# AvilaAndre/simgrid-flow-updating-implementation

Hardware: AMD Instinct MI355X
Metric: directed-edge flow updates/sec + % HBM roofline; rounds to 1e-9 error (higher is better)
Workload: dtype f64

## Files before the change

### simgrid-flow-updating-implementation_amd/csrc/fu_engine.hip

```cpp
#include <hip/hip_runtime.h>
#include <hip/hip_ext.h>

#include <algorithm>
#include <cmath>
#include <cstring>
#include <string>
#include <vector>

#include "fu_common.h"
#include "fu_plan.h"

using namespace fu;
namespace FP = fu::plan;

#define HIP_TRY(expr)                                                                     \
  do {                                                                                    \
    hipError_t _e = (expr);                                                               \
    if (_e != hipSuccess)                                                                 \
      return fu::fail(FU_ERR_HIP, std::string(#expr) + ": " + hipGetErrorString(_e));     \
  } while (0)

namespace {

using FP::kGeoEdges;
// ... 876 lines not shown
  const int excl = base + x - (len[0] + len[1]);
  if (2 * t < P) {
    s_m[2 * t] = excl;
    s_o[2 * t] = o[0];
  }
  if (2 * t + 1 < P) {
    s_m[2 * t + 1] = excl + len[0];
    s_o[2 * t + 1] = o[1];
  }
  if (t == 0) {
    int tot = 0;
    for (int k = 0; k < kTrThreads / 64; ++k) tot += s_w[k];
    s_m[P] = tot;
  }
  __syncthreads();
  const int nst = s_m[P];
  if (t < kTrBE / 64) {
    const int m = t * 64;
    int lo = 1, hi = P;
    while (lo < hi) {
      const int mid = (lo + hi) >> 1;
      if (s_m[mid] > m) hi = mid; else lo = mid + 1;
    }
    s_c[t] = lo;
  }
  if (t == 0) s_c[kTrBE / 64] = P;
  __syncthreads();
  constexpr int kPerT = kTrBE / kTrThreads;
  int g[kPerT];
#pragma unroll
  for (int k = 0; k < kPerT; ++k) {
    const int m = t + k * kTrThreads;
    g[k] = -1;
    if (m < nst) {
      int lo = s_c[m >> 6], hi = s_c[(m >> 6) + 1];
      while (lo < hi) {
        const int mid = (lo + hi) >> 1;
        if (s_m[mid] > m) hi = mid; else lo = mid + 1;
      }
      const int run = lo - 1;
      g[k] = s_o[run] + (m - s_m[run]);
    }
  }
  double val[kPerT];
  unsigned short pos[kPerT];
#pragma unroll
  for (int k = 0; k < kPerT; ++k) {
    val[k] = g[k] >= 0 ? GA[g[k]] : 0.0;
    pos[k] = g[k] >= 0 ? pos16[g[k]] : (unsigned short)0;
  }
  const int next = bk + nj;
  if (next < bend) load_runs(next, o, len);
#pragma unroll
  for (int k = 0; k < kPerT; ++k)
    if (g[k] >= 0) s_v[pos[k]] = val[k];
  __syncthreads();
  for (int q = t; q < ne; q += kTrThreads) {
    if constexpr (NT) __builtin_nontemporal_store(s_v[q], GB + e0 + q);
    else GB[e0 + q] = s_v[q];
  }
  if (next >= bend) break;
  __syncthreads();
  bk = next;
  }
}

__global__ __launch_bounds__(kBlock) void k_isolated(int i0, int n, const double *__restrict__ v,
                                                     double *__restrict__ a_new, const double *__restrict__ target,
                                                     unsigned long long *__restrict__ err, void *__restrict__ code_new,
                                                     PackCtl *__restrict__ ctl, int rslot, int check) {
  const PackCtl pc = ctl[2];
  if (blockIdx.x == 0 && threadIdx.x == 0) ctl[rslot] = pc;
  const int i = i0 + blockIdx.x * kBlock + threadIdx.x;
  unsigned long long eb = 0;
  if (i < n) {
    const double a = ((v[i] - 0.0) + 0.0) / (double)1;
    *(a_new + i) = a;
    if (pc.width) put_code(pc, code_new, i, a);
    if (check) eb = err_bits(a, target[i]);
  }
  if (check) block_max_to(eb, err);
}

template <bool CHECK, int TE, int TN, bool RF = true, bool LO = true>
__global__ __launch_bounds__(kBlock) void k_round_staged(
    const int4 *__restrict__ tiles, int t0, int ntl,
    const int *__restrict__ rowptr, const int *__restrict__ col,
    const StageArgs sa, const void *__restrict__ G, const double *__restrict__ v,
    double *__restrict__ F, const double *__restrict__ a_prev, const double *__restrict__ a_prev2,
    double *__restrict__ a_new, const double *__restrict__ target,
    unsigned long long *__restrict__ err, void *__restrict__ code_new, PackCtl *__restrict__ ctl,
    int rslot, int fm) {
  static_assert(TE % kBlock == 0 && TN <= kBlock, "tile geometry");
  static_assert(TE <= 1024, "the u16 staged index holds a 10-bit tile position");
  const PackCtl pp = ctl[rslot ^ 1];
  const int lsel = sa.sel[width_index(pp.width)];
  const PackCtl pc = ctl[2];
  if (blockIdx.x == 0 && threadIdx.x == 0) ctl[rslot] = pc;
  __shared__ double s_x[TE];
  __shared__ double s_er[TE];
  __shared__ unsigned char s_own[TE];
  __shared__ int s_rp[TN + 1];
  __shared__ double s_a[TN];
  const int t = threadIdx.x;
  unsigned long long eb = 0;
  const int xcd = blockIdx.x & 7, per = ntl >> 3, rem = ntl & 7;
  const int tile = t0 + xcd * per + min(xcd, rem) + (int)(blockIdx.x >> 3);
  const int4 tl = tiles[tile];
  const int nb = tl.x, nn = tl.y - tl.x;
  const int e0 = tl.z, ne = tl.w - tl.z;
  constexpr int kPer = TE / kBlock;
  const unsigned short *__restrict__ s16 = sa.sidx16[lsel];
  unsigned si[kPer];
  double x[kPer], g[kPer];
  int gi[kPer];
  int rp;
  double vv, own2;
  if constexpr (LO) {
  {
    const int dl = sa.dtab[lsel][(size_t)tile * kStageRuns + (t & 63)];
    unsigned short c16[kPer];
#pragma unroll
    for (int k = 0; k < kPer; ++k) {
      const int q = t + k * kBlock;
      const unsigned short c = s16[q < ne ? e0 + q : 0];
      c16[k] = q < ne ? c : (unsigned short)0;
    }
    if constexpr (RF) {
#pragma unroll
      for (int k = 0; k < kPer; ++k) {
        const int q = t + k * kBlock;
        const double f = ld_f(F, q < ne ? e0 + q : 0);
        x[k] = q < ne ? f : 0.0;
      }
    } else {
#pragma unroll
      for (int k = 0; k < kPer; ++k) x[k] = 0.0;
    }
    const int tn = min(t, nn - 1);
    const int rp0 = rowptr[nb + min(t, nn)];
    const double v0 = v[nb + tn], o0 = a_prev2[nb + tn];
    asm volatile("" ::: "memory");
    rp = t <= nn ? rp0 : 0;
    vv = t < nn ? v0 : 0.0;
    own2 = t < nn ? o0 : 0.0;
#pragma unroll
    for (int k = 0; k < kPer; ++k) {
      const int q = t + k * kBlock;
      const int dd = __shfl(dl, (int)(c16[k] >> 10));
      si[k] = c16[k] & 1023u;
      gi[k] = q < ne ? q + dd : -1;
    }
  }
  } else {
  {
    const int dl = sa.dtab[lsel][(size_t)tile * kStageRuns + (t & 63)];
    unsigned short c16[kPer];
#pragma unroll
    for (int k = 0; k < kPer; ++k) {
      const int q = t + k * kBlock;
      c16[k] = q < ne ? s16[e0 + q] : (unsigned short)0;
      x[k] = q < ne && RF ? ld_f(F, e0 + q) : 0.0;
    }
#pragma unroll
    for (int k = 0; k < kPer; ++k) {
      const int q = t + k * kBlock;
      const int dd = __shfl(dl, (int)(c16[k] >> 10));
      si[k] = c16[k] & 1023u;
      gi[k] = q < ne ? q + dd : -1;
    }
  }
  rp = t <= nn ? rowptr[nb + t] : 0;
  vv = t < nn ? v[nb + t] : 0.0;
  own2 = t < nn ? a_prev2[nb + t] : 0.0;
  }
  if (pp.width == 0) {
#pragma unroll
    for (int k = 0; k < kPer; ++k)
      g[k] = gi[k] >= 0 ? reinterpret_cast<const double *>(G)[gi[k]] : 0.0;
  } else {
    unsigned cd[kPer];
    unsigned esc;
    if (pp.width == 8) {
      esc = 0xFFu;
#pragma unroll
      for (int k = 0; k < kPer; ++k) cd[k] = gi[k] >= 0 ? reinterpret_cast<const unsigned char *>(G)[gi[k]] : 0u;
    } else if (pp.width == 16) {
      esc = 0xFFFFu;
#pragma unroll
      for (int k = 0; k < kPer; ++k) cd[k] = gi[k] >= 0 ? reinterpret_cast<const unsigned short *>(G)[gi[k]] : 0u;
    } else {
      esc = 0xFFFFFFFFu;
#pragma unroll
      for (int k = 0; k < kPer; ++k) cd[k] = gi[k] >= 0 ? reinterpret_cast<const unsigned *>(G)[gi[k]] : 0u;
    }
#pragma unroll
    for (int k = 0; k < kPer; ++k)
      g[k] = gi[k] < 0 ? 0.0 : cd[k] == esc ? a_prev[col[e0 + (int)(si[k] & 0xFFFFu)]] : dkey_inv(pp.base + cd[k]);
  }
#pragma unroll
  for (int k = 0; k < kPer; ++k) {
    const int q = t + k * kBlock;
    if (q < ne) {
      s_x[q] = x[k];
      s_er[si[k] & 0xFFFFu] = g[k];
    }
  }
  if (t <= nn) s_rp[t] = rp;
  __syncthreads();
  if (t < nn) {
    const int qb = s_rp[t] - e0, qe = s_rp[t + 1] - e0;
    double S = 0.0, T = 0.0;
    const double fo0 = fm ? old_flow(fm, own2) : 0.0;
    for (int q = qb; q < qe; ++q) {
      const double er = s_er[q];
      const double fr = recon_fr(fm ? fo0 : s_x[q], er, own2);
      s_x[q] = fr;
      s_own[q] = (unsigned char)t;
      S = S + fr;
      T = T + er;
    }
    const double a = ((vv - S) + T) / (double)(qe - qb + 1);
    s_a[t] = a;
    *(a_new + nb + t) = a;
    if (pc.width) put_code(pc, code_new, nb + t, a);
    if (CHECK) eb = err_bits(a, target[nb + t]);
  }
  __syncthreads();
#pragma unroll
  for (int k = 0; k < kPer; ++k) {
    const int q = t + k * kBlock;
    if (q < ne) {
      st_fo(F, e0 + q, (s_x[q] + s_a[s_own[q]]) - s_er[q], x[k], fm);
    }
  }
  if (CHECK) block_max_to(eb, err);
}


constexpr int kMCH = 64;
template <bool CHECK, int LAGM = 0>
__global__ __launch_bounds__(kBlock) void k_heavy_multi(
    const int *__restrict__ hrows, int nrows, const int *__restrict__ rowptr, const double *__restrict__ v,
    double *__restrict__ F, const double *__restrict__ a_prev2, double *__restrict__ a_new,
    const double *__restrict__ target, unsigned long long *__restrict__ err, void *__restrict__ code_new,
    PackCtl *__restrict__ ctl, const double *__restrict__ Gb, int fm,
    const double *__restrict__ Gb_old = nullptr, double *__restrict__ hist = nullptr) {
  constexpr bool LAG = LAGM > 0;
  constexpr bool mat = LAGM == 2;
  __shared__ double sh[2][2 * kMR][kMCH + 1];
  __shared__ int s_b[kMR], s_d[kMR];
  __shared__ double s_o2[kMR], s_a[kMR], s_o4[kMR];
  const PackCtl pc = ctl[2];
  const int t = threadIdx.x, w = t >> 6, lane = t & 63;
  const int r0 = blockIdx.x * kMR;
  if (t < kMR) {
    const bool ok = r0 + t < nrows;
    const int i = ok ? hrows[r0 + t] : 0;
    const int b = ok ? rowptr[i] : 0;
    s_b[t] = b;
    s_d[t] = ok ? rowptr[i + 1] - b : 0;
    const double o2 = ok ? a_prev2[i] : 0.0;
    s_o2[t] = o2;
    if (LAG) {
      s_o4[t] = ok && mat ? hist[r0 + t] : 0.0;
      if (ok) hist[r0 + t] = o2;
    }
  }
  __syncthreads();
  int rb[4], rd[4];
  double ro2[4], ro4[4];
#pragma unroll
  for (int j = 0; j < 4; ++j) {
    rb[j] = s_b[4 * w + j];
    rd[j] = s_d[4 * w + j];
    ro2[j] = s_o2[4 * w + j];
    ro4[j] = LAG ? s_o4[4 * w + j] : 0.0;
  }
  const int nch = (s_d[0] + kMCH - 1) / kMCH;
  double fo0[4], er0[4], fo1[4], er1[4];
  double eo0[4], eo1[4];
  auto load = [&](double (&fo)[4], double (&er)[4], double (&eo)[4], int c) {
#pragma unroll
    for (int j = 0; j < 4; ++j) {
      const int k = min(c * kMCH + lane, max(rd[j] - 1, 0));
      er[j] = Gb[rb[j] + k];
      if constexpr (mat) eo[j] = Gb_old[rb[j] + k];
      if constexpr (mat) fo[j] = ld_f(F, rb[j] + k);
      else fo[j] = ld_fo(F, rb[j] + k, fm, ro2[j]);
    }
  };
  auto put = [&](const double (&fo)[4], const double (&er)[4], const double (&eo)[4], int c, int buf) {
#pragma unroll
    for (int j = 0; j < 4; ++j) {
      const int r = 4 * w + j;
      const bool in = c * kMCH + lane < rd[j];
      double f2 = fo[j];
      if (LAG && in) {
        const int e = rb[j] + c * kMCH + lane;
        if constexpr (mat) {
          f2 = (recon_fr(fo[j], eo[j], ro4[j]) + ro2[j]) - eo[j];
          st_f(F, e, f2, fo[j]);
        } else if (fm) {
          st_f_full(F, e, f2);
        }
      }
      sh[buf][2 * r][lane] = in ? recon_fr(f2, er[j], ro2[j]) : 0.0;
      sh[buf][2 * r + 1][lane] = in ? er[j] : 0.0;
    }
  };
  const int cr = lane >> 1, ch = lane & 1;
  double acc = 0.0;
  auto chain = [&](int c, int buf) {
    if (w == 0 && lane < 2 * kMR) {
      const int len = min(kMCH, max(0, s_d[cr] - c * kMCH));
      const double *src = sh[buf][lane];
      int q = 0;
// ... 553 lines not shown
    if (++it > max_iters) {
      atomicExch(status, 1);
      break;
    }
  }
  if (done)
    while (sc < n_snap && snap_ticks[sc] < tick_end) snaps[(long long)sc++ * n + node] = lst;
#pragma unroll
  for (int j = 0; j < MAXD; ++j)
    if (j < deg) {
      flow[rb + j] = fl[j];
      est[rb + j] = es[j];
    }
  cursor[node] = p;
  scur[node] = sc;
  last[node] = lst;
}
#undef FU_RING_REFILL
#undef FU_RING_COMMIT
#undef FU_NEXT_RECVS


template <typename T>
int dmalloc(T **p, size_t count) {
  if (count == 0) count = 1;
  hipError_t e = hipMalloc((void **)p, sizeof(T) * count);
  if (e != hipSuccess) {
    *p = nullptr;
    return fail(FU_ERR_ALLOC, std::string("hipMalloc(") + std::to_string(sizeof(T) * count) + "): " + hipGetErrorString(e));
  }
  return FU_OK;
}

}

struct RoundCtx {
  int64_t r;
  int fm;
  double *F;
  const double *ap, *ap2;
  double *an;
  unsigned long long *err;
  bool plan;
};

constexpr int kPreMarks = 12;

struct fu_handle {
  int device = 0;
  std::vector<int32_t> h_new_of_old;
  std::vector<int64_t> h_orig_rowptr;
  hipStream_t stream = nullptr;
  hipStream_t stream2 = nullptr;
  hipEvent_t ev0 = nullptr, ev1 = nullptr;
  hipEvent_t ev2 = nullptr, ev3 = nullptr;
  hipEvent_t marks[64] = {};
  hipEvent_t r0_start = nullptr;
  hipEvent_t r0_stop = nullptr;
  hipEvent_t ev_pw = nullptr, ev_fork = nullptr, ev_join = nullptr;
  int32_t n = 0;
  int64_t E = 0;
  int32_t na = 0;
  int32_t max_deg = 0;
  int *rowptr = nullptr, *col = nullptr;
  int *blk_row = nullptr;
  unsigned short *col16 = nullptr;
  int *cbase = nullptr;
  std::vector<int32_t> h_cbase;
  double *v = nullptr;
  double *f[2] = {nullptr, nullptr};
  double *a[3] = {nullptr, nullptr, nullptr};
  double *target = nullptr;
  unsigned long long *err = nullptr;
  int errcap = 0;
  double *ftmp = nullptr;
  int64_t rounds = 0;
  int kernel = 4;
  int geo = 1;
  int hub_threshold = 128;
  int mega_hub = 8192;
  int wave_heavy = 1;
  int mid_heavy = 1;
  int tr_bpx = 32;
  int staged_lo = 1;
  int c16 = 1;
  int multi_mid = 1;
  int split_hubs = 1;
  int fork_heavy = 1;
  bool autotune = true;
  bool tuned = false;
  bool tune_for_width = false;
  bool tuning = false;
  float tune_ms[8] = {};
  int tune_out[8] = {};
  int n_tunes = 0;
  int tuned_width = 0;
  int tune_cache[4] = {-1, -1, -1, -1};
  int *h_pw = nullptr;
  void *h_xfer[2] = {nullptr, nullptr};
  hipEvent_t ev_xfer[2] = {nullptr, nullptr};
  bool pw_pending = false;
  int *pw_dev = nullptr;
  bool plan_pending = false;
  std::vector<int64_t> h_rowptr;
  std::vector<int32_t> h_col;
  int4 *tiles_geo[4] = {nullptr, nullptr, nullptr, nullptr};
  int *tnar_geo[4] = {nullptr, nullptr, nullptr, nullptr};
  int ntiles_geo[4] = {0, 0, 0, 0};
  int nheavy_geo[4] = {0, 0, 0, 0};
  int nbound_geo[4] = {0, 0, 0, 0};
  int niso_geo[4] = {0, 0, 0, 0};
  int iso0_geo[4] = {0, 0, 0, 0};
  FP::Tiles tiles1;
  int mid_geo[4][2] = {};
  int multi_geo[4][2] = {};
  int multi_heavy = 1;
  double *halo_a = nullptr;
  std::vector<int32_t> h_hrows;
  int *hrows = nullptr;
  int n_hub = 0;
  int64_t hub_total = 0;
  int4 *hub_rows = nullptr;
  int *hub_blk = nullptr;
  int iso_rows = 1;
  int multi_short = 1;
  int tr_nt = 1;
  int *hub_off = nullptr;
  double2 *hubxy = nullptr;
  unsigned char *code[2] = {nullptr, nullptr};
  PackCtl *pctl = nullptr;
  int *psample = nullptr;
  int n_psample = 0;
  int pack = 1;
  int pack_every = 16;
  int tile_edges = 1024;
  int tile_nodes = 0;
  bool has_target = false;
  struct StageLayout {
    int P = 0, Q = 0, SN = 0, NB = 0;
    int4 *brange = nullptr;
    unsigned short *colS = nullptr;
    unsigned short *sidx16 = nullptr;
    int *dtab = nullptr;
  };
  StageLayout st[4];
  bool st_ready = false;
  std::string st_why;
  int4 *st_tiles = nullptr;
  int st_ntiles = 0;
  int st_nbound = 0;
  int4 *st_heavy = nullptr;
  int st_nheavy = 0;
  void *stG = nullptr;
  int seen_width = 0;
  int st_force = -1;
  std::vector<FP::I4> h_light;
  struct TransLayout {
    int P = 0, Q = 0, NB = 0, B = 0;
    int Bh = 0;
    int Bm = 0;
    int4 *brange = nullptr;
    unsigned short *colS = nullptr;
    unsigned short *pos16 = nullptr;
    int *offT = nullptr;
    double *GA = nullptr;
    double *GBr[3] = {nullptr, nullptr, nullptr};
    double *hist[2] = {nullptr, nullptr};
// ... 218 lines not shown
  T.Bm = tp.Bm;
  h->tr_ready = true;
  return FU_OK;
}

inline unsigned grid_for(long long work) { return (unsigned)((work + kBlock - 1) / kBlock); }

int lag_finalize(fu_handle *h, int p) {
  if (!h->lagf[p]) return FU_OK;
  const int64_t rr = h->lag_round[p];
  if (h->rounds - rr < 1 || h->rounds - rr > 2)
    return fail(FU_ERR_STATE, "lag_finalize: lagged round " + std::to_string(rr) + " is not one of the last two (" +
                                  std::to_string(h->rounds) + " rounds done)");
  const double *Gb = h->tr.GBr[rr % 3];
  const double *a = h->a[rr % 3];
  if (h->lag_nmulti[p])
    hipLaunchKernelGGL(k_lag_final, dim3(h->lag_nmulti[p]), dim3(kBlock), 0, h->stream, h->hrows + h->multi_geo[1][0],
                       h->rowptr, h->f[p], Gb, h->tr.hist[p], a);
  HIP_TRY(hipGetLastError());
  h->lagf[p] = 0;
  return FU_OK;
}
int lag_finalize_all(fu_handle *h) {
  for (int p = 0; p < 2; ++p)
    if (int rc = lag_finalize(h, p)) return rc;
  return FU_OK;
}

inline unsigned tr_grid(fu_handle *h, int nbk) {
  const int per = (nbk + 7) / 8;
  return 8u * (unsigned)(h->tr_bpx > 0 ? std::min(per, h->tr_bpx) : per);
}


void plan_alone(fu_handle *h, RoundCtx &c) {
  if (!c.plan) return;
  hipLaunchKernelGGL(k_pack_plan, dim3(1), dim3(kBlock), 0, h->stream, c.ap, h->psample, h->pctl, h->pw_dev);
  c.plan = false;
}

int launch_round0(fu_handle *h, RoundCtx &c) {
  static_assert(sizeof(PackCtl) * 3 == 6 * sizeof(unsigned long long), "k_round0 clears 3 PackCtl");
  h->lagf[0] = h->lagf[1] = 0;
  if (h->r0_start) {
    hipExtLaunchKernelGGL(k_round0, dim3(grid_for(std::max(h->na, 6))), dim3(kBlock), 0, h->stream, h->r0_start,
                          h->r0_stop, 0, h->n, h->na, (const int *)h->rowptr, (const double *)h->v, h->a[0], h->a[2],
                          reinterpret_cast<unsigned long long *>(h->pctl));
    h->r0_start = h->r0_stop = nullptr;
  } else {
    hipLaunchKernelGGL(k_round0, dim3(grid_for(std::max(h->na, 6))), dim3(kBlock), 0, h->stream, h->n, h->na,
                       h->rowptr, h->v, h->a[0], h->a[2], reinterpret_cast<unsigned long long *>(h->pctl));
  }
  if (c.err)
    hipLaunchKernelGGL(k_max_err, dim3(std::min(1024u, grid_for(h->n))), dim3(kBlock), 0, h->stream, h->n,
                       h->a[0], h->target, c.err);
  if (h->dist) {
    h->halo_a = h->a[0];
    if (int rc = fu__dist_round_hook(h, 2)) return rc;
  }
  return FU_OK;
}

int launch_k8(fu_handle *h, RoundCtx &c) {
  constexpr bool C0 = false;
  const int r1 = (int)(c.r & 1);
  unsigned sgrid = 1;
  const StageArgs sa = stage_args(h, &sgrid);
  const void *cp = h->code[(c.r - 1) & 1];
  if (h->st_ntiles) {
    hipLaunchKernelGGL(k_stage, dim3(sgrid + (c.plan ? 8 : 0)), dim3(kStageThreads), 0, h->stream, sa, h->na, c.ap, cp,
                       h->pctl, r1, h->stG, c.plan ? h->psample : nullptr, h->pw_dev);
    c.plan = false;
  }
  plan_alone(h, c);
  auto heavy = [&](auto chk) {
    hipLaunchKernelGGL((k_round_recon<decltype(chk)::value, kStageTE, kStageTN>), dim3(h->st_nheavy),
                       dim3(kBlock), 0, h->stream, h->st_heavy, h->rowptr, h->col, h->v, c.F, c.ap, c.ap2, c.an,
                       h->target, c.err, cp, h->code[r1], h->pctl, r1, nullptr, nullptr, nullptr, 0, nullptr, c.fm);
  };
  if (h->st_nheavy) {
    if (c.err) heavy(std::true_type{});
    else heavy(std::false_type{});
  }
  auto light = [&](auto chk, auto rf, auto lo) -> int {
    const int nb = h->dist ? h->st_nbound : 0;
    for (int part = 0; part < 2; ++part) {
      const int t0 = part ? nb : 0, cnt = part ? h->st_ntiles - nb : nb;
      if (cnt)
        hipLaunchKernelGGL((k_round_staged<decltype(chk)::value, kStageTE, kStageTN, decltype(rf)::value,
                                           decltype(lo)::value>),
                           dim3(cnt), dim3(kBlock), 0, h->stream, h->st_tiles, t0, cnt, h->rowptr, h->col, sa,
                           h->stG, h->v, c.F, c.ap, c.ap2, c.an, h->target, c.err, h->code[r1], h->pctl, r1, c.fm);
      if (!part && h->dist) {
        h->halo_a = c.an;
        if (int rc = fu__dist_round_hook(h, 2)) return rc;
      }
    }
    return FU_OK;
  };
  auto light_lo = [&](auto chk, auto rf) {
    return h->staged_lo ? light(chk, rf, std::true_type{}) : light(chk, rf, std::false_type{});
  };
  auto light_rf = [&](auto chk) {
    return c.fm ? light_lo(chk, std::false_type{}) : light_lo(chk, std::true_type{});
  };
  if (h->st_ntiles || h->dist) {
    if (c.err) return light_rf(std::true_type{});
    return light_rf(std::integral_constant<bool, C0>{});
  }
  return FU_OK;
}

int launch_k9(fu_handle *h, RoundCtx &c) {
  if (int rc = ensure_transpose(h)) return rc;
  double *Gb = h->tr.GBr[c.r % 3];
  const double *Gb_old = h->tr.GBr[(c.r + 1) % 3];
  if (!Gb) return fail(FU_ERR_STATE, "kernel 9: no pre-gather buffer");
  const int r1 = (int)(c.r & 1);
  const void *cp = h->code[(c.r - 1) & 1];
  FP::K9Opts ko;
  ko.mid_heavy = h->mid_heavy;
  ko.multi_mid = h->multi_mid;
  ko.multi_short = h->multi_short;
  ko.multi_heavy = h->multi_heavy;
  ko.wave_heavy = h->wave_heavy;
  ko.iso_rows = h->iso_rows;
  const FP::K9Sched ks = FP::k9_schedule(h->tiles1, h->n_hub, ko);
  const int nmega = ks.nmega, nh = ks.nh, niso = ks.niso, nl = ks.nl, m0 = ks.m0, m1 = ks.m1;
  const int4 *tl = h->tiles_geo[1];
  const bool hubs = nmega > 0;
  const int n_multi = ks.n_multi, m1s = ks.m1s;
  const bool multi = ks.multi;
  const bool lag_multi = h->lag && multi;
  const int p = r1;
  if (h->lagf[p] && h->lag_nmulti[p] != (lag_multi ? n_multi : 0)) {
    if (int rc = lag_finalize(h, p)) return rc;
  }
  const int lagm = lag_multi ? (h->lagf[p] ? 2 : 1) : 0;
  StageArgs sa{};
  for (int li = 0; li < 4; ++li) sa.sel[li] = 3;
  sa.P[3] = h->tr.P;
  sa.Q[3] = h->tr.Q;
  sa.SN[3] = kStageLds / 8;
  sa.NB[3] = h->tr.NB;
  sa.brange[3] = h->tr.brange;
  sa.colS[3] = h->tr.colS;
  sa.f64 = 1;
  {
    hipLaunchKernelGGL(k_stage, dim3(h->tr.NB + (c.plan ? 8 : 0)), dim3(kStageThreads), 0, h->stream, sa, h->na, c.ap,
                       cp, h->pctl, r1, h->tr.GA, c.plan ? h->psample : nullptr, h->pw_dev);
    c.plan = false;
  }
  plan_alone(h, c);
  const int bh = hubs ? h->tr.Bh : 0;
  auto tr_launch = [&](int b0, int nb) {
    if (h->tr_nt)
      hipLaunchKernelGGL(k_transpose<true>, dim3(tr_grid(h, nb)), dim3(kTrThreads), 0, h->stream, b0, nb, h->tr.P,
                         (long long)h->E, h->tr.offT, h->tr.GA, h->tr.pos16, Gb);
    else
      hipLaunchKernelGGL(k_transpose<false>, dim3(tr_grid(h, nb)), dim3(kTrThreads), 0, h->stream, b0, nb, h->tr.P,
                         (long long)h->E, h->tr.offT, h->tr.GA, h->tr.pos16, Gb);
  };
  if (bh) tr_launch(0, bh);
  if (hubs) {
    HIP_TRY(hipEventRecord(h->ev_fork, h->stream));
    HIP_TRY(hipStreamWaitEvent(h->stream2, h->ev_fork, 0));
  }
  if (h->tr.B > bh) tr_launch(bh, h->tr.B - bh);
  const bool chk = c.err != nullptr;
  if (hubs) {
    auto chains = [&](auto C) {
      hipLaunchKernelGGL((k_round_recon<decltype(C)::value, 1024, 128, 2, true>), dim3(nmega), dim3(kBlock),
                         0, h->stream2, tl, h->rowptr, h->col, h->v, c.F, c.ap, c.ap2, c.an, h->target, c.err, cp,
                         h->code[r1], h->pctl, r1, nullptr, nullptr, h->hrows, 1, Gb, c.fm);
    };
    if (chk) chains(std::true_type{});
    else chains(std::false_type{});
    hipLaunchKernelGGL(k_hub_flows, dim3(grid_for(h->hub_total)), dim3(kBlock), 0, h->stream2, h->n_hub, h->hub_rows,
                       (long long)h->hub_total, nullptr, c.an, c.F, Gb, c.ap2, c.fm, h->hub_blk);
    HIP_TRY(hipGetLastError());
    HIP_TRY(hipEventRecord(h->ev_join, h->stream2));
  }
  auto heavy = [&](auto C, auto RL, int t0, int t1) {
    if (t1 > t0)
      hipLaunchKernelGGL((k_round_recon<decltype(C)::value, 1024, 128, 2, true, decltype(RL)::value>),
                         dim3(t1 - t0), dim3(kBlock), 0, h->stream, tl + t0, h->rowptr, h->col, h->v, c.F, c.ap, c.ap2,
                         c.an, h->target, c.err, cp, h->code[r1], h->pctl, r1, h->hubxy, h->hub_off, h->hrows, 1, Gb,
// ... 321 lines not shown
  FU_TRY_BEGIN
  if (!g || !value || !out || layout < 0 || layout > 1) return fail(FU_ERR_ARG, "fu_create_from_graph_ex: bad arguments");
  if (layout == 0) return fu_create_from_graph(g, value, device, out);
  const int32_t n = g->n;
  std::vector<int32_t> nofo(n);
  fu_graph *rg = nullptr;
  if (int rc = fu_graph_relabel(g, 1, nofo.data(), &rg)) return rc;
  std::vector<double> v2(n);
  for (int32_t i = 0; i < n; ++i) v2[nofo[i]] = value[i];
  const int rc = fu_create_from_graph(rg, v2.data(), device, out);
  fu_graph_free(rg);
  if (rc) return rc;
  (*out)->h_new_of_old.swap(nofo);
  (*out)->h_orig_rowptr = g->rowptr;
  return FU_OK;
  FU_TRY_END
}

int fu_set_option(fu_handle *h, const char *key, int64_t value) {
  FU_TRY_BEGIN
  if (!h || !key) return fail(FU_ERR_ARG, "fu_set_option: NULL argument");
  if (int rc = set_device(h)) return rc;
  if (!std::strcmp(key, "kernel")) {
    if (value != 0 && value != 4 && value != 8 && value != 9)
      return fail(FU_ERR_ARG, "fu_set_option: kernel must be 0 (auto), 4 (recon), 8 (stage) or 9 (pregather)");
    if (h->rounds != 0) return fail(FU_ERR_STATE, "fu_set_option: kernel can only change before the first round (call fu_reset)");
    int rc = FU_OK;
    if (value == 8) rc = ensure_stage(h);
    if (value == 9) rc = ensure_transpose(h);
    if (h->dist) {
      const std::string why = rc ? fu_last_error() : "";
      int all_ok = 1;
      if (int rc2 = fu__dist_agree(h, rc == FU_OK, &all_ok)) return rc2;
      if (rc) return fail(rc, why);
      if (!all_ok) return fail(FU_ERR_STATE, "fu_set_option: kernel " + std::to_string(value) + " failed on another rank");
    }
    if (rc) return rc;
    if (value == 9) h->geo = 1;
    h->kernel = value == 0 ? 4 : (int)value;
    h->autotune = value == 0;
    h->tuned = false;
    h->tune_for_width = false;
    return FU_OK;
  }
  if (!std::strcmp(key, "stage_layout")) {
    if (value < -1 || value > 3) return fail(FU_ERR_ARG, "fu_set_option: stage_layout must be -1..3");
    h->st_force = (int)value;
    return FU_OK;
  }
  if (!std::strcmp(key, "pack")) {
    h->pack = value != 0;
    if (!h->pack) {
      h->plan_pending = false;
      HIP_TRY(hipMemsetAsync(h->pctl + 2, 0, sizeof(PackCtl), h->stream));
    }
    return FU_OK;
  }
  if (!std::strcmp(key, "pack_every")) {
    if (value < 1 || value > (1 << 20)) return fail(FU_ERR_ARG, "fu_set_option: pack_every must be in [1, 2^20]");
    h->pack_every = (int)value;
    return FU_OK;
  }
  if (!std::strcmp(key, "tile_edges")) {
    if (value != 2048 && value != 1024 && value != 512) return fail(FU_ERR_ARG, "fu_set_option: tile_edges must be 2048, 1024 or 512");
    h->tile_edges = (int)value;
    h->geo = h->tile_edges == 2048 ? 0 : h->tile_edges == 512 ? 3 : h->tile_nodes == 256 ? 2 : 1;
    return FU_OK;
  }
  if (!std::strcmp(key, "tile_nodes")) {
    if (value != 0 && value != 128 && value != 256) return fail(FU_ERR_ARG, "fu_set_option: tile_nodes must be 0, 128 or 256");
    h->tile_nodes = (int)value;
    h->geo = h->tile_edges == 2048 ? 0 : h->tile_edges == 512 ? 3 : h->tile_nodes == 256 ? 2 : 1;
    return FU_OK;
  }
  if (!std::strcmp(key, "fork_heavy")) {
    h->fork_heavy = value != 0;
    return FU_OK;
  }
  if (!std::strcmp(key, "split_hubs")) {
    h->split_hubs = value != 0;
    return FU_OK;
  }
  if (!std::strcmp(key, "staged_lo")) {
    h->staged_lo = value != 0;
    return FU_OK;
  }
  if (!std::strcmp(key, "tr_bpx")) {
    if (value < 0 || value > 1 << 20) return fail(FU_ERR_ARG, "fu_set_option: tr_bpx must be in [0, 2^20]");
    h->tr_bpx = (int)value;
    return FU_OK;
  }
  if (!std::strcmp(key, "lag")) {
    const int lv = value != 0;
    if (lv != h->lag) {
      if (int rc = lag_finalize_all(h)) return rc;
      free_transpose(h);
      h->lag = lv;
    }
    return FU_OK;
  }
  if (!std::strcmp(key, "tr_nt")) {
    if (value != 0 && value != 1) return fail(FU_ERR_ARG, "fu_set_option: tr_nt must be 0 or 1");
    h->tr_nt = (int)value;
    return FU_OK;
  }
  if (!std::strcmp(key, "multi_short")) {
    h->multi_short = value != 0;
    return FU_OK;
  }
  if (!std::strcmp(key, "iso_rows")) {
    h->iso_rows = value != 0;
    return FU_OK;
  }
  if (!std::strcmp(key, "multi_heavy")) {
    h->multi_heavy = value != 0;
    return FU_OK;
  }
  if (!std::strcmp(key, "c16")) {
    h->c16 = value != 0;
    return FU_OK;
  }
  if (!std::strcmp(key, "multi_mid")) {
    h->multi_mid = value != 0;
    return FU_OK;
  }
  if (!std::strcmp(key, "mid_heavy")) {
    h->mid_heavy = value != 0;
    return FU_OK;
  }
  if (!std::strcmp(key, "wave_heavy")) {
    h->wave_heavy = value != 0;
    return build_tiles(h);
  }
  if (!std::strcmp(key, "mega_hub")) {
    if (value < 1) return fail(FU_ERR_ARG, "fu_set_option: mega_hub must be >= 1");
    h->mega_hub = (int)std::min<int64_t>(value, INT32_MAX);
    return build_tiles(h);
  }
  if (!std::strcmp(key, "hub_threshold")) {
    if (value < 1) return fail(FU_ERR_ARG, "fu_set_option: hub_threshold must be >= 1");
    if (h->st_tiles) return fail(FU_ERR_STATE, "fu_set_option: hub_threshold must be set before kernel 8 is prepared");
    h->hub_threshold = (int)std::min<int64_t>(value, 2048);
    return build_tiles(h);
  }
  return fail(FU_ERR_ARG, std::string("fu_set_option: unknown key '") + key + "'");
  FU_TRY_END
}

int fu_reset(fu_handle *h) {
  FU_TRY_BEGIN
  if (!h) return fail(FU_ERR_ARG, "fu_reset: NULL handle");
  if (int rc = set_device(h)) return rc;
  if (h->dist) {
    if (int rc = fu__dist_round_hook(h, 1)) return rc;
  }
  HIP_TRY(hipStreamSynchronize(h->stream));
  h->rounds = 0;
  h->lagf[0] = h->lagf[1] = 0;
  h->pw_pending = false;
  h->plan_pending = false;
  *h->h_pw = 0;
  h->seen_width = 0;
  if (h->autotune && (h->tuned || h->tune_for_width) && h->tune_cache[0] >= 0) {
    use_cand(h, kCands[h->tune_cache[0]]);
    h->tuned_width = 0;
    h->tuned = true;
    h->tune_for_width = false;
// ... 898 lines not shown
```

Before: 200.5 billion.

## Vectorize staged-round flow I/O as quad-aligned hi/lo word loads and stores

The staged round kernel now gives each lane a contiguous aligned quad of edges, so flow loads and stores become 128-bit accesses over the split hi/lo word layout. A tail element handles the misalignment, and high words are written only when they change, which cuts write traffic. Packed code gathers are unified into a single 32-bit word load plus a shift, replacing the per-width branches. The staged_lo variant and its option are removed. This adds alignment bookkeeping and relies on the fhi_idx layout placing 4 consecutive edges contiguously.

```diff
diff --git a/simgrid-flow-updating-implementation_amd/csrc/fu_engine.hip b/simgrid-flow-updating-implementation_amd/csrc/fu_engine.hip
--- a/simgrid-flow-updating-implementation_amd/csrc/fu_engine.hip
+++ b/simgrid-flow-updating-implementation_amd/csrc/fu_engine.hip
@@ -982,24 +982,24 @@
   if (check) block_max_to(eb, err);
 }
 
-template <bool CHECK, int TE, int TN, bool RF = true, bool LO = true>
+template <bool CHECK, int TE, int TN, bool RF = true>
 __global__ __launch_bounds__(kBlock) void k_round_staged(
     const int4 *__restrict__ tiles, int t0, int ntl,
     const int *__restrict__ rowptr, const int *__restrict__ col,
     const StageArgs sa, const void *__restrict__ G, const double *__restrict__ v,
-    double *__restrict__ F, const double *__restrict__ a_prev, const double *__restrict__ a_prev2,
+    double *F, const double *__restrict__ a_prev, const double *__restrict__ a_prev2,
     double *__restrict__ a_new, const double *__restrict__ target,
     unsigned long long *__restrict__ err, void *__restrict__ code_new, PackCtl *__restrict__ ctl,
     int rslot, int fm) {
-  static_assert(TE % kBlock == 0 && TN <= kBlock, "tile geometry");
+  static_assert(TE == 4 * kBlock && TN <= kBlock, "tile geometry: one quad of edges per lane");
   static_assert(TE <= 1024, "the u16 staged index holds a 10-bit tile position");
   const PackCtl pp = ctl[rslot ^ 1];
   const int lsel = sa.sel[width_index(pp.width)];
   const PackCtl pc = ctl[2];
   if (blockIdx.x == 0 && threadIdx.x == 0) ctl[rslot] = pc;
-  __shared__ double s_x[TE];
-  __shared__ double s_er[TE];
-  __shared__ unsigned char s_own[TE];
+  __shared__ __align__(16) double s_x[TE + 4];
+  __shared__ __align__(16) double s_er[TE + 4];
+  __shared__ __align__(4) unsigned char s_own[TE + 4];
   __shared__ int s_rp[TN + 1];
   __shared__ double s_a[TN];
   const int t = threadIdx.x;
@@ -1009,33 +1009,45 @@
   const int4 tl = tiles[tile];
   const int nb = tl.x, nn = tl.y - tl.x;
   const int e0 = tl.z, ne = tl.w - tl.z;
-  constexpr int kPer = TE / kBlock;
   const unsigned short *__restrict__ s16 = sa.sidx16[lsel];
-  unsigned si[kPer];
-  double x[kPer], g[kPer];
-  int gi[kPer];
+  unsigned *fo = reinterpret_cast<unsigned *>(F);
+  const unsigned *fw = fo;
+  const int r = e0 & 3, eq0 = e0 - r, pe = r + ne;
+  const int p0 = 4 * t;
+  bool ok[4];
+#pragma unroll
+  for (int u = 0; u < 4; ++u) ok[u] = p0 + u >= r && p0 + u < pe;
+  const bool any = ne > 0 && p0 + 3 >= r && p0 < pe;
+  const bool full = p0 >= r && p0 + 3 < pe;
+  const int eq = any ? eq0 + p0 : 0;
+  const bool tok = TE + t < pe;
+  const int et = eq0 + TE + t;
+  unsigned si[4];
+  double g[4];
+  uint4 hq = make_uint4(0u, 0u, 0u, 0u), lq = hq;
+  unsigned hwt = 0u, lwt = 0u;
+  int gi[4];
   int rp;
   double vv, own2;
-  if constexpr (LO) {
   {
+    if constexpr (RF) {
+      if (tok) {
+        const long long i = fhi_idx(et);
+        hwt = fw[i];
+        lwt = fw[i + 32];
+      }
+    }
     const int dl = sa.dtab[lsel][(size_t)tile * kStageRuns + (t & 63)];
-    unsigned short c16[kPer];
-#pragma unroll
-    for (int k = 0; k < kPer; ++k) {
+    unsigned c16[4];
+#pragma unroll
+    for (int k = 0; k < 4; ++k) {
       const int q = t + k * kBlock;
-      const unsigned short c = s16[q < ne ? e0 + q : 0];
-      c16[k] = q < ne ? c : (unsigned short)0;
+      c16[k] = s16[q < ne ? e0 + q : 0];
     }
     if constexpr (RF) {
-#pragma unroll
-      for (int k = 0; k < kPer; ++k) {
-        const int q = t + k * kBlock;
-        const double f = ld_f(F, q < ne ? e0 + q : 0);
-        x[k] = q < ne ? f : 0.0;
-      }
-    } else {
-#pragma unroll
-      for (int k = 0; k < kPer; ++k) x[k] = 0.0;
+      const long long i = fhi_idx(eq);
+      hq = *reinterpret_cast<const uint4 *>(fw + i);
+      lq = *reinterpret_cast<const uint4 *>(fw + i + 32);
     }
     const int tn = min(t, nn - 1);
     const int rp0 = rowptr[nb + min(t, nn)];
@@ -1045,71 +1057,57 @@
     vv = t < nn ? v0 : 0.0;
     own2 = t < nn ? o0 : 0.0;
 #pragma unroll
-    for (int k = 0; k < kPer; ++k) {
+    for (int k = 0; k < 4; ++k) {
       const int q = t + k * kBlock;
       const int dd = __shfl(dl, (int)(c16[k] >> 10));
       si[k] = c16[k] & 1023u;
       gi[k] = q < ne ? q + dd : -1;
     }
   }
+  if (pp.width == 0) {
+#pragma unroll
+    for (int u = 0; u < 4; ++u) {
+      const double d = reinterpret_cast<const double *>(G)[max(gi[u], 0)];
+      g[u] = gi[u] >= 0 ? d : 0.0;
+    }
   } else {
-  {
-    const int dl = sa.dtab[lsel][(size_t)tile * kStageRuns + (t & 63)];
-    unsigned short c16[kPer];
-#pragma unroll
-    for (int k = 0; k < kPer; ++k) {
-      const int q = t + k * kBlock;
-      c16[k] = q < ne ? s16[e0 + q] : (unsigned short)0;
-      x[k] = q < ne && RF ? ld_f(F, e0 + q) : 0.0;
-    }
-#pragma unroll
-    for (int k = 0; k < kPer; ++k) {
-      const int q = t + k * kBlock;
-      const int dd = __shfl(dl, (int)(c16[k] >> 10));
-      si[k] = c16[k] & 1023u;
-      gi[k] = q < ne ? q + dd : -1;
-    }
-  }
-  rp = t <= nn ? rowptr[nb + t] : 0;
-  vv = t < nn ? v[nb + t] : 0.0;
-  own2 = t < nn ? a_prev2[nb + t] : 0.0;
-  }
-  if (pp.width == 0) {
-#pragma unroll
-    for (int k = 0; k < kPer; ++k)
-      g[k] = gi[k] >= 0 ? reinterpret_cast<const double *>(G)[gi[k]] : 0.0;
+    const int lb = pp.width == 8 ? 0 : pp.width == 16 ? 1 : 2;
+    const unsigned esc = 0xFFFFFFFFu >> (32 - pp.width);
+    const char *Gc = reinterpret_cast<const char *>(G);
+    auto ld_word = [&](int i) {
+      const size_t b = (size_t)max(i, 0) << lb;
+      return *reinterpret_cast<const unsigned *>(Gc + (b & ~(size_t)3));
+    };
+    auto code_of = [&](unsigned w, int i) { return (w >> ((((unsigned)max(i, 0) << lb) & 3u) * 8u)) & esc; };
+    unsigned cd[4];
+#pragma unroll
+    for (int u = 0; u < 4; ++u) cd[u] = ld_word(gi[u]);
+#pragma unroll
+    for (int u = 0; u < 4; ++u) {
+      cd[u] = code_of(cd[u], gi[u]);
+      g[u] = gi[u] < 0 ? 0.0 : cd[u] == esc ? a_prev[col[e0 + (int)si[u]]] : dkey_inv(pp.base + cd[u]);
+    }
+  }
+  const unsigned hw[4] = {hq.x, hq.y, hq.z, hq.w}, lw[4] = {lq.x, lq.y, lq.z, lq.w};
+  double x[4];
+#pragma unroll
+  for (int u = 0; u < 4; ++u) x[u] = __hiloint2double((int)hw[u], (int)lw[u]);
+  if (full) {
+    *reinterpret_cast<double2 *>(&s_x[p0]) = make_double2(x[0], x[1]);
+    *reinterpret_cast<double2 *>(&s_x[p0 + 2]) = make_double2(x[2], x[3]);
   } else {
-    unsigned cd[kPer];
-    unsigned esc;
-    if (pp.width == 8) {
-      esc = 0xFFu;
-#pragma unroll
-      for (int k = 0; k < kPer; ++k) cd[k] = gi[k] >= 0 ? reinterpret_cast<const unsigned char *>(G)[gi[k]] : 0u;
-    } else if (pp.width == 16) {
-      esc = 0xFFFFu;
-#pragma unroll
-      for (int k = 0; k < kPer; ++k) cd[k] = gi[k] >= 0 ? reinterpret_cast<const unsigned short *>(G)[gi[k]] : 0u;
-    } else {
-      esc = 0xFFFFFFFFu;
-#pragma unroll
-      for (int k = 0; k < kPer; ++k) cd[k] = gi[k] >= 0 ? reinterpret_cast<const unsigned *>(G)[gi[k]] : 0u;
-    }
-#pragma unroll
-    for (int k = 0; k < kPer; ++k)
-      g[k] = gi[k] < 0 ? 0.0 : cd[k] == esc ? a_prev[col[e0 + (int)(si[k] & 0xFFFFu)]] : dkey_inv(pp.base + cd[k]);
-  }
-#pragma unroll
-  for (int k = 0; k < kPer; ++k) {
-    const int q = t + k * kBlock;
-    if (q < ne) {
-      s_x[q] = x[k];
-      s_er[si[k] & 0xFFFFu] = g[k];
-    }
-  }
+#pragma unroll
+    for (int u = 0; u < 4; ++u)
+      if (ok[u]) s_x[p0 + u] = x[u];
+  }
+#pragma unroll
+  for (int k = 0; k < 4; ++k)
+    if (gi[k] >= 0) s_er[r + (int)si[k]] = g[k];
+  if (tok) s_x[TE + t] = __hiloint2double((int)hwt, (int)lwt);
   if (t <= nn) s_rp[t] = rp;
   __syncthreads();
   if (t < nn) {
-    const int qb = s_rp[t] - e0, qe = s_rp[t + 1] - e0;
+    const int qb = s_rp[t] - eq0, qe = s_rp[t + 1] - eq0;
     double S = 0.0, T = 0.0;
     const double fo0 = fm ? old_flow(fm, own2) : 0.0;
     for (int q = qb; q < qe; ++q) {
@@ -1127,12 +1125,45 @@
     if (CHECK) eb = err_bits(a, target[nb + t]);
   }
   __syncthreads();
-#pragma unroll
-  for (int k = 0; k < kPer; ++k) {
-    const int q = t + k * kBlock;
-    if (q < ne) {
-      st_fo(F, e0 + q, (s_x[q] + s_a[s_own[q]]) - s_er[q], x[k], fm);
-    }
+  if (any) {
+    const double2 xa = *reinterpret_cast<const double2 *>(&s_x[p0]), xb = *reinterpret_cast<const double2 *>(&s_x[p0 + 2]);
+    const double2 ea = *reinterpret_cast<const double2 *>(&s_er[p0]), ec = *reinterpret_cast<const double2 *>(&s_er[p0 + 2]);
+    const unsigned ow = *reinterpret_cast<const unsigned *>(&s_own[p0]);
+    const double xs[4] = {xa.x, xa.y, xb.x, xb.y}, es[4] = {ea.x, ea.y, ec.x, ec.y};
+    unsigned nh[4], nl[4];
+    bool ch[4];
+#pragma unroll
+    for (int u = 0; u < 4; ++u) {
+      const int own = ok[u] ? (int)((ow >> (8 * u)) & 0xFFu) : 0;
+      const double f = (xs[u] + s_a[own]) - es[u];
+      nh[u] = (unsigned)__double2hiint(f);
+      nl[u] = (unsigned)__double2loint(f);
+      ch[u] = !RF || fm || nh[u] != hw[u];
+    }
+    unsigned *w = fo + fhi_idx(eq);
+    if (full) {
+      *reinterpret_cast<uint4 *>(w + 32) = make_uint4(nl[0], nl[1], nl[2], nl[3]);
+      if (ch[0] && ch[1] && ch[2] && ch[3]) {
+        *reinterpret_cast<uint4 *>(w) = make_uint4(nh[0], nh[1], nh[2], nh[3]);
+      } else {
+#pragma unroll
+        for (int u = 0; u < 4; ++u)
+          if (ch[u]) st_fw(w + u, nh[u]);
+      }
+    } else {
+#pragma unroll
+      for (int u = 0; u < 4; ++u)
+        if (ok[u]) {
+          st_fw(w + 32 + u, nl[u]);
+          if (ch[u]) st_fw(w + u, nh[u]);
+        }
+    }
+  }
+  if (tok) {
+    const double f = (s_x[TE + t] + s_a[s_own[TE + t]]) - s_er[TE + t];
+    unsigned *w = fo + fhi_idx(et);
+    st_fw(w + 32, (unsigned)__double2loint(f));
+    if (!RF || fm || (unsigned)__double2hiint(f) != hwt) st_fw(w, (unsigned)__double2hiint(f));
   }
   if (CHECK) block_max_to(eb, err);
 }
@@ -1852,7 +1883,6 @@
   int wave_heavy = 1;
   int mid_heavy = 1;
   int tr_bpx = 32;
-  int staged_lo = 1;
   int c16 = 1;
   int multi_mid = 1;
   int split_hubs = 1;
@@ -2237,13 +2267,12 @@
     if (c.err) heavy(std::true_type{});
     else heavy(std::false_type{});
   }
-  auto light = [&](auto chk, auto rf, auto lo) -> int {
+  auto light = [&](auto chk, auto rf) -> int {
     const int nb = h->dist ? h->st_nbound : 0;
     for (int part = 0; part < 2; ++part) {
       const int t0 = part ? nb : 0, cnt = part ? h->st_ntiles - nb : nb;
       if (cnt)
-        hipLaunchKernelGGL((k_round_staged<decltype(chk)::value, kStageTE, kStageTN, decltype(rf)::value,
-                                           decltype(lo)::value>),
+        hipLaunchKernelGGL((k_round_staged<decltype(chk)::value, kStageTE, kStageTN, decltype(rf)::value>),
                            dim3(cnt), dim3(kBlock), 0, h->stream, h->st_tiles, t0, cnt, h->rowptr, h->col, sa,
                            h->stG, h->v, c.F, c.ap, c.ap2, c.an, h->target, c.err, h->code[r1], h->pctl, r1, c.fm);
       if (!part && h->dist) {
@@ -2253,11 +2282,8 @@
     }
     return FU_OK;
   };
-  auto light_lo = [&](auto chk, auto rf) {
-    return h->staged_lo ? light(chk, rf, std::true_type{}) : light(chk, rf, std::false_type{});
-  };
   auto light_rf = [&](auto chk) {
-    return c.fm ? light_lo(chk, std::false_type{}) : light_lo(chk, std::true_type{});
+    return c.fm ? light(chk, std::false_type{}) : light(chk, std::true_type{});
   };
   if (h->st_ntiles || h->dist) {
     if (c.err) return light_rf(std::true_type{});
@@ -2745,7 +2771,6 @@
     return FU_OK;
   }
   if (!std::strcmp(key, "staged_lo")) {
-    h->staged_lo = value != 0;
     return FU_OK;
   }
   if (!std::strcmp(key, "tr_bpx")) {
```

After: 206.6 billion, median of 6. 3.0% higher.
